# EdoardoBotta/RQ-VAE-Recommender

Measured on AMD Instinct MI355X. Metric: item-embeddings quantized/sec (RQ-VAE fwd+bwd), higher is better.
Workload: dtype f32 (MLP GEMMs f16x2-emulated)

## Files before the change

rq-vae-recommender_amd/csrc/gemm_split.hip:

```cpp
#include "rqhip_common.h"

namespace rqhip {

typedef float gs_f32x16 __attribute__((ext_vector_type(16)));
typedef float gs_f32x4 __attribute__((ext_vector_type(4)));
typedef float gs_f32x2 __attribute__((ext_vector_type(2)));
typedef __bf16 gs_bf16x8 __attribute__((ext_vector_type(8)));
typedef __bf16 gs_bf16x2 __attribute__((ext_vector_type(2)));
typedef _Float16 gs_f16x8 __attribute__((ext_vector_type(8)));
typedef _Float16 gs_f16x2 __attribute__((ext_vector_type(2)));
typedef unsigned gs_u32x2 __attribute__((ext_vector_type(2)));
typedef unsigned gs_u32x4 __attribute__((ext_vector_type(4)));
typedef int gs_i32x4 __attribute__((ext_vector_type(4)));

constexpr int kGsUB = 2;
constexpr int kGsK = 16;
constexpr int kGsColmaxLds = 1024;
constexpr int kGsTailWords = kWeightImageTailWords;

__device__ __forceinline__ void gs_split2(float a, float b, unsigned &h, unsigned &m, unsigned &l) {
    const gs_bf16x2 hh = __builtin_convertvector(gs_f32x2{a, b}, gs_bf16x2);
    h = __builtin_bit_cast(unsigned, hh);
    const float ra = a - __builtin_bit_cast(float, h << 16), rb = b - __builtin_bit_cast(float, h & 0xffff0000u);
    const gs_bf16x2 mm = __builtin_convertvector(gs_f32x2{ra, rb}, gs_bf16x2);
    m = __builtin_bit_cast(unsigned, mm);
    const float sa = ra - __builtin_bit_cast(float, m << 16), sb = rb - __builtin_bit_cast(float, m & 0xffff0000u);
    const gs_bf16x2 ll = __builtin_convertvector(gs_f32x2{sa, sb}, gs_bf16x2);
    l = __builtin_bit_cast(unsigned, ll);
}
__device__ __forceinline__ void gs_split2_f16(float a, float b, unsigned &h, unsigned &m) {
    const gs_f16x2 hh = __builtin_convertvector(gs_f32x2{a, b}, gs_f16x2);
    h = __builtin_bit_cast(unsigned, hh);
    const gs_f32x2 hf = __builtin_convertvector(hh, gs_f32x2);
    const gs_f16x2 mm = __builtin_convertvector(gs_f32x2{a - hf.x, b - hf.y}, gs_f16x2);
    m = __builtin_bit_cast(unsigned, mm);
}
constexpr int kGsF16Top = 14;
__device__ __forceinline__ int gs_exp_of_bits(unsigned b) {
    b &= 0x7fffffffu;
    const int e = (int)(b >> 23);
    return (b == 0u || e == 255) ? 0 : (e == 0 ? -126 : e - 127) - kGsF16Top;
}
__device__ __forceinline__ unsigned gs_abs_bits(float v) { return __builtin_bit_cast(unsigned, v) & 0x7fffffffu; }
__device__ __forceinline__ unsigned gs_umax(unsigned a, unsigned b) { return a > b ? a : b; }
__device__ __forceinline__ unsigned gs_half_wave_umax(unsigned v) {
    v = gs_umax(v, (unsigned)__builtin_amdgcn_update_dpp(0, (int)v, 0x111, 0xf, 0xf, true));
    v = gs_umax(v, (unsigned)__builtin_amdgcn_update_dpp(0, (int)v, 0x112, 0xf, 0xf, true));
    v = gs_umax(v, (unsigned)__builtin_amdgcn_update_dpp(0, (int)v, 0x114, 0xf, 0xf, true));
    v = gs_umax(v, (unsigned)__builtin_amdgcn_update_dpp(0, (int)v, 0x118, 0xf, 0xf, true));
    v = gs_umax(v, (unsigned)__builtin_amdgcn_update_dpp(0, (int)v, 0x142, 0xa, 0xf, true));
    return v;
}

constexpr int kImgCols = 4;
constexpr int kImgMaxJobs = 16;
struct ImageJob {
    const float *src;
    unsigned *image;
    int Nc, R, transpose, np;
    int block0;
};
struct ImageJobs {
    ImageJob j[kImgMaxJobs];
    int n;
};

__global__ __launch_bounds__(256) void weight_images_kernel(const ImageJobs jobs) {
    int ji = 0;
#pragma unroll 1
    for (int i = 1; i < jobs.n; ++i)
        if ((int)blockIdx.x >= jobs.j[i].block0) ji = i;
    const ImageJob job = jobs.j[ji];
    const int blk = (int)blockIdx.x - job.block0;
    const int Nc = job.Nc, R = job.R, np = job.np, n0 = blk * kImgCols;
    unsigned *tail = job.image + (size_t)(R / kGsK) * 2 * np * Nc * 4;
    if (blk == 0 && threadIdx.x < kGsTailWords) tail[threadIdx.x] = 0u;
    __shared__ unsigned s_max[kImgCols];
    if (threadIdx.x < kImgCols) s_max[threadIdx.x] = 0u;
    __syncthreads();
    const int pairs = R / 2, total = kImgCols * pairs;
    auto locate = [&](int idx, int &nl, int &rp) {
        if (job.transpose) { nl = idx % kImgCols; rp = idx / kImgCols; }
        else { rp = idx % pairs; nl = idx / pairs; }
    };
    auto fetch = [&](int nl, int rp, float &a, float &b) {
        const int n = n0 + nl, r = 2 * rp;
        a = job.transpose ? job.src[(size_t)r * Nc + n] : job.src[(size_t)n * R + r];
        b = job.transpose ? job.src[(size_t)(r + 1) * Nc + n] : job.src[(size_t)n * R + r + 1];
    };
    if (np == 2) {
        if (job.transpose) {
            __shared__ unsigned s_part[256];
            const int nl = threadIdx.x % kImgCols;
            unsigned m = 0u;
            for (int r = threadIdx.x / kImgCols; r < R; r += 256 / kImgCols) m = gs_umax(m, gs_abs_bits(job.src[(size_t)r * Nc + n0 + nl]));
            s_part[threadIdx.x] = m;
            __syncthreads();
            if (threadIdx.x < kImgCols) {
                for (int i = threadIdx.x + kImgCols; i < 256; i += kImgCols) m = gs_umax(m, s_part[i]);
                s_max[threadIdx.x] = m;
            }
        } else {
            const int lane = threadIdx.x & 63, nl = threadIdx.x >> 6;
            unsigned m = 0u;
            for (int rp = lane; rp < pairs; rp += 64) {
                const gs_f32x2 v = *reinterpret_cast<const gs_f32x2 *>(job.src + (size_t)(n0 + nl) * R + 2 * rp);
                m = gs_umax(m, gs_umax(gs_abs_bits(v.x), gs_abs_bits(v.y)));
            }
#pragma unroll
            for (int o = 32; o > 0; o >>= 1) m = gs_umax(m, (unsigned)__shfl_xor((int)m, o, 64));
            if (lane == 0) s_max[nl] = m;
        }
        __syncthreads();
        if (threadIdx.x < kImgCols) reinterpret_cast<int *>(tail + kGsTailWords)[n0 + threadIdx.x] = gs_exp_of_bits(s_max[threadIdx.x]);
    }
    for (int idx = threadIdx.x; idx < total; idx += 256) {
        int nl, rp;
        float a, b;
        locate(idx, nl, rp);
        fetch(nl, rp, a, b);
        const int n = n0 + nl, r = 2 * rp;
        unsigned h, m, l = 0u;
        if (np == 2) {
            const int e = gs_exp_of_bits(s_max[nl]);
            gs_split2_f16(ldexpf(a, -e), ldexpf(b, -e), h, m);
        } else {
            gs_split2(a, b, h, m, l);
        }
        const int s = r >> 4, half = (r >> 3) & 1, j2 = (r & 7) >> 1;
        const size_t base = ((size_t)(s * np) * 2 + half) * Nc + n;
        job.image[(base + 0 * 2 * (size_t)Nc) * 4 + j2] = h;
        job.image[(base + 1 * 2 * (size_t)Nc) * 4 + j2] = m;
        if (np == 3) job.image[(base + 2 * 2 * (size_t)Nc) * 4 + j2] = l;
    }
}

__global__ __launch_bounds__(256) void maxima_kernel(const float *__restrict__ A, const float *__restrict__ Y, float *__restrict__ out,
                                                     long long M, int R, unsigned *__restrict__ row_max, unsigned *__restrict__ col_max) {
    extern __shared__ unsigned mx_smem[];
    const int lane = threadIdx.x & 63, wave = threadIdx.x >> 6;
    if (col_max) {
        for (int c = threadIdx.x; c < R; c += 256) mx_smem[c] = 0u;
        __syncthreads();
    }
    constexpr int kQ = 4;
    for (int c0 = 0; c0 < R; c0 += 256 * kQ) {
    const int R4 = (R - c0 < 256 * kQ ? R - c0 : 256 * kQ) / 4;
    unsigned cm[kQ][4];
#pragma unroll
    for (int q = 0; q < kQ; ++q)
#pragma unroll
        for (int j = 0; j < 4; ++j) cm[q][j] = 0u;
    for (long long row = (long long)blockIdx.x * 4 + wave; row < M; row += (long long)gridDim.x * 4) {
        const gs_f32x4 *src = reinterpret_cast<const gs_f32x4 *>(A + (size_t)row * R + c0);
        const gs_f32x4 *ys = Y ? reinterpret_cast<const gs_f32x4 *>(Y + (size_t)row * R + c0) : nullptr;
        gs_f32x4 *dst = out ? reinterpret_cast<gs_f32x4 *>(out + (size_t)row * R + c0) : nullptr;
        unsigned rm = 0u;
#pragma unroll
        for (int q = 0; q < kQ; ++q) {
            const int i = lane + 64 * q;
            if (i >= R4) break;
            gs_f32x4 v = src[i];
            if (ys) {
                const gs_f32x4 y4 = ys[i];
                v.x = y4.x <= 0.0f ? 0.0f : v.x; v.y = y4.y <= 0.0f ? 0.0f : v.y;
                v.z = y4.z <= 0.0f ? 0.0f : v.z; v.w = y4.w <= 0.0f ? 0.0f : v.w;
                if (dst) dst[i] = v;
            }
#pragma unroll
            for (int j = 0; j < 4; ++j) {
                const unsigned b = gs_abs_bits(v[j]);
                rm = gs_umax(rm, b);
                cm[q][j] = gs_umax(cm[q][j], b);
            }
        }
        if (row_max) {
#pragma unroll
            for (int o = 32; o > 0; o >>= 1) rm = gs_umax(rm, (unsigned)__shfl_xor((int)rm, o, 64));
            if (lane == 0) row_max[row] = c0 == 0 ? rm : gs_umax(rm, row_max[row]);
        }
    }
    if (col_max) {
#pragma unroll
        for (int q = 0; q < kQ; ++q) {
            const int i = lane + 64 * q;
            if (i >= R4) break;
#pragma unroll
            for (int j = 0; j < 4; ++j) atomicMax(&mx_smem[c0 + 4 * i + j], cm[q][j]);
        }
    }
    }
    if (col_max) {
        __syncthreads();
        for (int c = threadIdx.x; c < R; c += 256)
            if (mx_smem[c]) atomicMax(col_max + c, mx_smem[c]);
    }
}

struct GemmSplitParams {
    const float *A;
    const unsigned *planes;
    float *C;
    long long M;
    int R, Nc;
    int n_col_tiles;
    unsigned n_big, n_tiles;
    int rt_big;
    unsigned *counter;
    int n_queues;
    int rt_fastest;
    int static_tiles;
    const float *X;
    float *rowsum;
    float row_scale;
    const unsigned *a_max;
    int a_parts;
    const int *b_exp;
    unsigned *c_rowmax, *c_colmax;
};

#ifndef GS_PROBE
#define GS_PROBE 0
#endif
#ifndef GS_PROLOGUE_ORDER
#define GS_PROLOGUE_ORDER 1
#endif
#ifndef GS_FAST_EPILOGUE
#define GS_FAST_EPILOGUE 1
#endif
#ifndef GS_REGION_PAD
#define GS_REGION_PAD 32
#endif

__device__ __forceinline__ unsigned gs_row16_umax(unsigned v) {
    v = gs_umax(v, (unsigned)__builtin_amdgcn_update_dpp(0, (int)v, 0x111, 0xf, 0xf, true));
    v = gs_umax(v, (unsigned)__builtin_amdgcn_update_dpp(0, (int)v, 0x112, 0xf, 0xf, true));
    v = gs_umax(v, (unsigned)__builtin_amdgcn_update_dpp(0, (int)v, 0x114, 0xf, 0xf, true));
    v = gs_umax(v, (unsigned)__builtin_amdgcn_update_dpp(0, (int)v, 0x118, 0xf, 0xf, true));
    return v;
}
__device__ __forceinline__ float gs_row16_sum(float v) {
    v = v + __builtin_bit_cast(float, __builtin_amdgcn_update_dpp(0, __builtin_bit_cast(int, v), 0x111, 0xf, 0xf, true));
    v = v + __builtin_bit_cast(float, __builtin_amdgcn_update_dpp(0, __builtin_bit_cast(int, v), 0x112, 0xf, 0xf, true));
    v = v + __builtin_bit_cast(float, __builtin_amdgcn_update_dpp(0, __builtin_bit_cast(int, v), 0x114, 0xf, 0xf, true));
    v = v + __builtin_bit_cast(float, __builtin_amdgcn_update_dpp(0, __builtin_bit_cast(int, v), 0x118, 0xf, 0xf, true));
    return v;
}

constexpr int kGsTS = 68;
__host__ __device__ constexpr size_t gs_epilogue_lds(int waves, int rows, int wn) { return (size_t)waves * 32 * kGsTS * 4 + (size_t)2 * wn * rows * 4; }

template <int EPI, int TA, int COLS, int NP, int WAVES>
__device__ __forceinline__ void gs_epilogue(const GemmSplitParams &p, gs_f32x16 (&acc)[TA][kGsUB], unsigned *sbuf, const int *s_aexp,
                                            unsigned *s_colmax, long long m0, int n0) {
    constexpr int kGsThreads = 64 * WAVES;
    constexpr int UB = kGsUB, WN = COLS / (32 * UB), WM = WAVES / WN, ROWS = WM * 32 * TA;
    static_assert(UB == 2, "a wave's tile is 64 columns wide");
    int tid = threadIdx.x;
    asm volatile("" : "+v"(tid));
    const int lane = tid & 63, wave = tid >> 6;
    const int il = lane & 31, h = lane >> 5;
    const int wm = wave / WN, wn = wave % WN;
    const int cl = lane & 15, rl = lane >> 4;
    float *tb = reinterpret_cast<float *>(sbuf) + (size_t)wave * 32 * kGsTS;
    float *red = reinterpret_cast<float *>(sbuf) + (size_t)WAVES * 32 * kGsTS;
    unsigned *mred = reinterpret_cast<unsigned *>(red) + WN * ROWS;
    const bool want_rowmax = p.c_rowmax != nullptr, want_colmax = p.c_colmax != nullptr;
    const int colw = n0 + 64 * wn + 4 * cl;
    gs_i32x4 ec = {0, 0, 0, 0};
    if (NP == 2) ec = *reinterpret_cast<const gs_i32x4 *>(p.b_exp + colw);
    unsigned cmx[4] = {0u, 0u, 0u, 0u};
#if GS_FAST_EPILOGUE
    if (NP == 2 && want_rowmax && want_colmax && m0 + ROWS <= p.M) {
        const size_t row0 = (size_t)(m0 + 32 * TA * wm + rl);
        float *cbase = p.C + row0 * p.Nc + colw;
        const float *xbase = EPI >= 2 ? p.X + row0 * p.Nc + colw : nullptr;
        unsigned *pad = reinterpret_cast<unsigned *>(tb) + il * kGsTS + 64 + h;
        gs_f32x4 xn[8];
        if (EPI >= 2) {
#pragma unroll
            for (int k = 0; k < 8; ++k) xn[k] = *reinterpret_cast<const gs_f32x4 *>(xbase + (size_t)(4 * k) * p.Nc);
        }
#pragma unroll
        for (int t = 0; t < TA; ++t) {
#pragma unroll
            for (int u = 0; u < UB; ++u)
#pragma unroll
                for (int g = 0; g < 4; ++g)
                    *reinterpret_cast<gs_f32x4 *>(tb + il * kGsTS + 32 * u + 8 * g + 4 * h) =
                        gs_f32x4{acc[t][u][4 * g], acc[t][u][4 * g + 1], acc[t][u][4 * g + 2], acc[t][u][4 * g + 3]};
            __builtin_amdgcn_fence(__ATOMIC_RELEASE, "wavefront");
            __builtin_amdgcn_wave_barrier();
            gs_f32x4 v8[8], x8[8];
            int er8[8];
#pragma unroll
            for (int k = 0; k < 8; ++k) {
                v8[k] = *reinterpret_cast<const gs_f32x4 *>(tb + (4 * k + rl) * kGsTS + 4 * cl);
                er8[k] = s_aexp[32 * TA * wm + 32 * t + 4 * k + rl];
            }
            if (EPI >= 2) {
#pragma unroll
                for (int k = 0; k < 8; ++k) x8[k] = xn[k];
                if (t + 1 < TA) {
#pragma unroll
                    for (int k = 0; k < 8; ++k) xn[k] = *reinterpret_cast<const gs_f32x4 *>(xbase + (size_t)(32 * (t + 1) + 4 * k) * p.Nc);
                }
            }
#pragma unroll
            for (int k = 0; k < 8; ++k) {
                const int rloc = 32 * TA * wm + 32 * t + 4 * k + rl;
                gs_f32x4 v = v8[k];
#pragma unroll
                for (int j = 0; j < 4; ++j) v[j] = ldexpf(v[j], er8[k] + ec[j]);
                const gs_f32x4 x4 = EPI >= 2 ? x8[k] : gs_f32x4{0.f, 0.f, 0.f, 0.f};
                if (EPI == 1) {
                    v.x = v.x < 0.0f ? 0.0f : v.x; v.y = v.y < 0.0f ? 0.0f : v.y;
                    v.z = v.z < 0.0f ? 0.0f : v.z; v.w = v.w < 0.0f ? 0.0f : v.w;
                }
                float sq = 0.0f;
                if (EPI == 2) {
#pragma unroll
                    for (int j = 0; j < 4; ++j) {
                        const float d = v[j] - x4[j];
                        sq = sq + d * d;
                        v[j] = (2.0f * d) * p.row_scale;
                    }
                }
                if (EPI == 3) {
                    v.x = x4.x <= 0.0f ? 0.0f : v.x; v.y = x4.y <= 0.0f ? 0.0f : v.y;
                    v.z = x4.z <= 0.0f ? 0.0f : v.z; v.w = x4.w <= 0.0f ? 0.0f : v.w;
                }
                unsigned rmx = 0u;
#pragma unroll
                for (int j = 0; j < 4; ++j) {
                    const unsigned bb = gs_abs_bits(v[j]);
                    rmx = gs_umax(rmx, bb);
                    cmx[j] = gs_umax(cmx[j], bb);
                }
                *reinterpret_cast<gs_f32x4 *>(cbase + (size_t)(32 * t + 4 * k) * p.Nc) = v;
                if (EPI == 2) {
                    const float s16 = gs_row16_sum(sq);
                    float *dst = cl == 15 ? red + wn * ROWS + rloc : reinterpret_cast<float *>(pad);
                    *dst = s16;
                }
                const unsigned m16 = gs_row16_umax(rmx);
                unsigned *dstm = cl == 15 ? mred + wn * ROWS + rloc : pad;
                *dstm = m16;
            }
            __builtin_amdgcn_fence(__ATOMIC_RELEASE, "wavefront");
            __builtin_amdgcn_wave_barrier();
        }
    } else
#endif
    {
    constexpr int kAux = 4, NQ = 8 * TA;
    gs_f32x4 xa[kAux];
    auto aux_of = [&](int q) {
        long long r = m0 + 32 * TA * wm + 4 * q + rl;
        r = r < p.M ? r : p.M - 1;
        return *reinterpret_cast<const gs_f32x4 *>(p.X + (size_t)r * p.Nc + colw);
    };
    if (EPI >= 2) {
#pragma unroll
        for (int q = 0; q < kAux; ++q) xa[q] = aux_of(q);
    }
#pragma unroll
    for (int t = 0; t < TA; ++t) {
#pragma unroll
        for (int u = 0; u < UB; ++u)
#pragma unroll
            for (int g = 0; g < 4; ++g)
                *reinterpret_cast<gs_f32x4 *>(tb + il * kGsTS + 32 * u + 8 * g + 4 * h) =
                    gs_f32x4{acc[t][u][4 * g], acc[t][u][4 * g + 1], acc[t][u][4 * g + 2], acc[t][u][4 * g + 3]};
        __builtin_amdgcn_fence(__ATOMIC_RELEASE, "wavefront");
        __builtin_amdgcn_wave_barrier();
#pragma unroll
        for (int k = 0; k < 8; ++k) {
            const int q = 8 * t + k;
            const int rloc = 32 * TA * wm + 32 * t + 4 * k + rl;
            const long long grow = m0 + rloc;
            gs_f32x4 v = *reinterpret_cast<const gs_f32x4 *>(tb + (4 * k + rl) * kGsTS + 4 * cl);
            if (NP == 2) {
                const int er = s_aexp[rloc];
#pragma unroll
                for (int j = 0; j < 4; ++j) v[j] = ldexpf(v[j], er + ec[j]);
            }
            gs_f32x4 x4 = {0.f, 0.f, 0.f, 0.f};
            if (EPI >= 2) {
                x4 = xa[q % kAux];
                if (q + kAux < NQ) xa[q % kAux] = aux_of(q + kAux);
            }
            if (EPI == 1) {
                v.x = v.x < 0.0f ? 0.0f : v.x; v.y = v.y < 0.0f ? 0.0f : v.y;
                v.z = v.z < 0.0f ? 0.0f : v.z; v.w = v.w < 0.0f ? 0.0f : v.w;
            }
            float sq = 0.0f;
            if (EPI == 2) {
#pragma unroll
                for (int j = 0; j < 4; ++j) {
                    const float d = v[j] - x4[j];
                    sq = sq + d * d;
                    v[j] = (2.0f * d) * p.row_scale;
                }
            }
            if (EPI == 3) {
                v.x = x4.x <= 0.0f ? 0.0f : v.x; v.y = x4.y <= 0.0f ? 0.0f : v.y;
                v.z = x4.z <= 0.0f ? 0.0f : v.z; v.w = x4.w <= 0.0f ? 0.0f : v.w;
            }
            unsigned rmx = 0u;
            if (grow < p.M) {
                if (want_rowmax | want_colmax) {
#pragma unroll
                    for (int j = 0; j < 4; ++j) {
                        const unsigned bb = gs_abs_bits(v[j]);
                        rmx = gs_umax(rmx, bb);
                        cmx[j] = gs_umax(cmx[j], bb);
                    }
                }
                *reinterpret_cast<gs_f32x4 *>(p.C + (size_t)grow * p.Nc + colw) = v;
            }
            if (EPI == 2) {
                const float s16 = gs_row16_sum(sq);
                if (cl == 15) red[wn * ROWS + rloc] = s16;
            }
            if (want_rowmax) {
                const unsigned m16 = gs_row16_umax(rmx);
                if (cl == 15) mred[wn * ROWS + rloc] = m16;
            }
        }
        __builtin_amdgcn_fence(__ATOMIC_RELEASE, "wavefront");
        __builtin_amdgcn_wave_barrier();
    }
    }
    if (want_colmax) {
#pragma unroll
        for (int j = 0; j < 4; ++j) {
            unsigned m = gs_umax(cmx[j], (unsigned)__shfl_xor((int)cmx[j], 16, 64));
            m = gs_umax(m, (unsigned)__shfl_xor((int)m, 32, 64));
            if (rl == 0 && m != 0u) {
                if (p.Nc <= kGsColmaxLds) atomicMax(&s_colmax[colw + j], m);
                else atomicMax(p.c_colmax + colw + j, m);
            }
        }
    }
    if (want_rowmax || EPI == 2) {
        __syncthreads();
        if (want_rowmax) {
            unsigned *dst = p.c_rowmax + (size_t)(n0 / (COLS > 256 ? 256 : COLS)) * p.M;
            for (int r = tid; r < ROWS; r += kGsThreads) {
                if (m0 + r >= p.M) continue;
                unsigned mx = mred[r];
#pragma unroll
                for (int w = 1; w < WN; ++w) mx = gs_umax(mx, mred[w * ROWS + r]);
                dst[m0 + r] = mx;
                if (COLS > 256) dst[p.M + m0 + r] = mx;
            }
        }
        if (EPI == 2) {
            for (int r = tid; r < ROWS; r += kGsThreads) {
                if (m0 + r >= p.M) continue;
                float sum = red[r];
#pragma unroll
                for (int w = 1; w < WN; ++w) sum = sum + red[w * ROWS + r];
                p.rowsum[(size_t)(n0 / COLS) * p.M + m0 + r] = sum;
            }
        }
    }
}

template <int EPI, int TA, int COLS, int NP, int WAVES>
__device__ __forceinline__ void gs_tile(const GemmSplitParams &p, unsigned *sbuf, int *s_aexp, unsigned *s_colmax, long long m0, int n0) {
    constexpr int kGsWaves = WAVES, kGsThreads = 64 * WAVES;
    constexpr int UB = kGsUB, WN = COLS / (32 * UB), WM = kGsWaves / WN;
    constexpr int ROWS = WM * 32 * TA, AQ = (ROWS * 4 + kGsThreads - 1) / kGsThreads;
    constexpr int PA = NP * 2 * ROWS * 4, PB = NP * 2 * COLS * 4;
    constexpr int BQ = (2 * NP * COLS + kGsThreads - 1) / kGsThreads;
    const int tid = threadIdx.x, lane = tid & 63, wave = tid >> 6;
    const int il = lane & 31, h = lane >> 5;
    const int wm = wave / WN, wn = wave % WN;
    const int n_stage = p.R / kGsK;
    constexpr int APASS = kGsThreads / 4;
    const int arow = tid >> 2, akq = tid & 3;
    constexpr bool kAllLive = (ROWS * 4) % kGsThreads == 0;
    bool a_live[AQ];
    const float *asrc[AQ];
    int a_e[AQ];
#pragma unroll
    for (int q = 0; q < AQ; ++q) {
        a_live[q] = kAllLive || arow + APASS * q < ROWS;
        long long arow_g = m0 + arow + APASS * q;
        arow_g = arow_g < p.M ? arow_g : p.M - 1;
        asrc[q] = p.A + (size_t)arow_g * p.R + 4 * akq;
        a_e[q] = 0;
        if (NP == 2) {
            unsigned mx = 0u;
            const unsigned *am = p.a_max + arow_g;
            for (int part = 0; part < p.a_parts; part += 4) {
                unsigned v[4];
#pragma unroll
                for (int j = 0; j < 4; ++j) v[j] = am[(size_t)(part + j < p.a_parts ? part + j : part) * p.M];
                mx = gs_umax(gs_umax(mx, gs_umax(v[0], v[1])), gs_umax(v[2], v[3]));
            }
            a_e[q] = gs_exp_of_bits(mx);
            if (a_live[q] && akq == 0) s_aexp[arow + APASS * q] = a_e[q];
        }
    }

    gs_f32x16 acc[TA][UB];
#pragma unroll
    for (int t = 0; t < TA; ++t)
#pragma unroll
        for (int u = 0; u < UB; ++u)
#pragma unroll
            for (int r = 0; r < 16; ++r) acc[t][u][r] = 0.0f;

    gs_f32x4 ra0[AQ], ra1[AQ];
    gs_u32x4 rb[BQ];
    auto fetchA = [&](int stage, gs_f32x4 *dst) {
        stage = stage < n_stage ? stage : n_stage - 1;
#pragma unroll
        for (int q = 0; q < AQ; ++q) dst[q] = *reinterpret_cast<const gs_f32x4 *>(asrc[q] + stage * kGsK);
    };
    auto fetchB = [&](int stage) {
        stage = stage < n_stage ? stage : n_stage - 1;
        const gs_u32x4 *img = reinterpret_cast<const gs_u32x4 *>(p.planes) + (size_t)stage * 2 * NP * p.Nc + n0;
#pragma unroll
        for (int q = 0; q < BQ; ++q) {
            const int e = tid + kGsThreads * q;
            if ((2 * NP * COLS) % kGsThreads != 0 && e >= 2 * NP * COLS) continue;
            rb[q] = img[(size_t)(e / COLS) * p.Nc + (e % COLS)];
        }
    };
    auto stash = [&](int buf, const gs_f32x4 *ra) {
        unsigned *dA = sbuf + buf * (PA + PB), *dB = dA + PA;
#pragma unroll
        for (int q = 0; q < AQ; ++q) {
            if (!kAllLive && !a_live[q]) continue;
            unsigned h01, m01, l01 = 0u, h23, m23, l23 = 0u;
            if (NP == 2) {
                gs_split2_f16(ldexpf(ra[q].x, -a_e[q]), ldexpf(ra[q].y, -a_e[q]), h01, m01);
                gs_split2_f16(ldexpf(ra[q].z, -a_e[q]), ldexpf(ra[q].w, -a_e[q]), h23, m23);
            } else {
                gs_split2(ra[q].x, ra[q].y, h01, m01, l01);
                gs_split2(ra[q].z, ra[q].w, h23, m23, l23);
            }
            unsigned *d = dA + (((akq >> 1) * ROWS) + arow + APASS * q) * 4 + 2 * (akq & 1);
            *reinterpret_cast<gs_u32x2 *>(d + 0 * 2 * ROWS * 4) = gs_u32x2{h01, h23};
            *reinterpret_cast<gs_u32x2 *>(d + 1 * 2 * ROWS * 4) = gs_u32x2{m01, m23};
            if (NP == 3) *reinterpret_cast<gs_u32x2 *>(d + 2 * 2 * ROWS * 4) = gs_u32x2{l01, l23};
        }
#pragma unroll
        for (int q = 0; q < BQ; ++q) {
            const int e = tid + kGsThreads * q;
            if ((2 * NP * COLS) % kGsThreads != 0 && e >= 2 * NP * COLS) continue;
            *reinterpret_cast<gs_u32x4 *>(dB + (size_t)e * 4) = rb[q];
        }
    };
    auto multiply = [&](int buf) {
        const gs_bf16x8 *aA = reinterpret_cast<const gs_bf16x8 *>(sbuf + buf * (PA + PB));
        const gs_bf16x8 *bB = reinterpret_cast<const gs_bf16x8 *>(sbuf + buf * (PA + PB) + PA);
        if constexpr (NP == 2) {
            gs_f16x8 fb[UB][2];
#pragma unroll
            for (int u = 0; u < UB; ++u)
#pragma unroll
                for (int pc = 0; pc < 2; ++pc)
                    fb[u][pc] = __builtin_bit_cast(gs_f16x8, bB[(pc * 2 + h) * COLS + wn * 32 * UB + 32 * u + il]);
#pragma unroll
            for (int t = 0; t < TA; ++t) {
                gs_f16x8 fa[2];
#pragma unroll
                for (int pc = 0; pc < 2; ++pc)
                    fa[pc] = __builtin_bit_cast(gs_f16x8, aA[(pc * 2 + h) * ROWS + wm * 32 * TA + 32 * t + il]);
#pragma unroll
                for (int u = 0; u < UB; ++u) {
                    gs_f32x16 c16 = acc[t][u];
                    c16 = __builtin_amdgcn_mfma_f32_32x32x16_f16(fb[u][0], fa[1], c16, 0, 0, 0);
                    c16 = __builtin_amdgcn_mfma_f32_32x32x16_f16(fb[u][1], fa[0], c16, 0, 0, 0);
                    c16 = __builtin_amdgcn_mfma_f32_32x32x16_f16(fb[u][0], fa[0], c16, 0, 0, 0);
                    acc[t][u] = c16;
                }
            }
        } else {
#pragma unroll
            for (int u = 0; u < UB; ++u) {
                gs_bf16x8 b[3];
#pragma unroll
                for (int pc = 0; pc < 3; ++pc) b[pc] = bB[(pc * 2 + h) * COLS + wn * 32 * UB + 32 * u + il];
#pragma unroll
                for (int t = 0; t < TA; ++t) {
                    gs_bf16x8 a[3];
#pragma unroll
                    for (int pc = 0; pc < 3; ++pc) a[pc] = aA[(pc * 2 + h) * ROWS + wm * 32 * TA + 32 * t + il];
                    gs_f32x16 c16 = acc[t][u];
                    c16 = __builtin_amdgcn_mfma_f32_32x32x16_bf16(b[1], a[1], c16, 0, 0, 0);
                    c16 = __builtin_amdgcn_mfma_f32_32x32x16_bf16(b[0], a[2], c16, 0, 0, 0);
                    c16 = __builtin_amdgcn_mfma_f32_32x32x16_bf16(b[2], a[0], c16, 0, 0, 0);
                    c16 = __builtin_amdgcn_mfma_f32_32x32x16_bf16(b[0], a[1], c16, 0, 0, 0);
                    c16 = __builtin_amdgcn_mfma_f32_32x32x16_bf16(b[1], a[0], c16, 0, 0, 0);
                    c16 = __builtin_amdgcn_mfma_f32_32x32x16_bf16(b[0], a[0], c16, 0, 0, 0);
                    acc[t][u] = c16;
                }
            }
        }
    };

#if GS_PROLOGUE_ORDER
    gs_f32x4 rp[AQ];
    fetchA(0, rp);
    fetchB(0);
    __builtin_amdgcn_sched_barrier(0);
    fetchA(1, ra1);
    __builtin_amdgcn_sched_barrier(0);
    stash(0, rp);
    __builtin_amdgcn_sched_barrier(0);
    fetchB(1);
    __builtin_amdgcn_sched_barrier(0);
    fetchA(2, ra0);
    __builtin_amdgcn_sched_barrier(0);
    __syncthreads();
#else
    fetchA(0, ra0);
    fetchB(0);
    fetchA(1, ra1);
    stash(0, ra0);
    fetchB(1);
    fetchA(2, ra0);
    __syncthreads();
#endif
    const int n_pair = n_stage & ~1;
    for (int c = 0; c < n_pair; c += 2) {
        stash(1, ra1);
        fetchB(c + 2);
        fetchA(c + 3, ra1);
        multiply(0);
        __syncthreads();
        stash(0, ra0);
        fetchB(c + 3);
        fetchA(c + 4, ra0);
        multiply(1);
        __syncthreads();
    }
    if (n_stage & 1) {
        multiply(0);
        __syncthreads();
    }

    gs_epilogue<EPI, TA, COLS, NP, WAVES>(p, acc, sbuf, s_aexp, s_colmax, m0, n0);
}

template <int EPI, int TA, int COLS = 256>
__device__ __forceinline__ void gs_tile2(const GemmSplitParams &p, unsigned *sbuf, int *s_aexp, unsigned *s_colmax, long long m0, int n0) {
    constexpr int WAVES = COLS / 64, UB = kGsUB, kThreads = 64 * WAVES;
    constexpr int ROWS = 32 * TA;
    constexpr int AQ = (ROWS * 4 + kThreads - 1) / kThreads;
    constexpr bool kAllLive = (ROWS * 4) % kThreads == 0;
    constexpr int kRegion = ROWS * 4 + GS_REGION_PAD;
    constexpr int PA = 4 * kRegion;
    const int tid = threadIdx.x, lane = tid & 63, wn = tid >> 6;
    const int il = lane & 31, h = lane >> 5;
    const int n_stage = p.R / kGsK;
    constexpr int APASS = kThreads / 4;
    const int arow = tid >> 2, akq = tid & 3;
    const float *asrc[AQ];
    int a_e[AQ];
    bool a_live[AQ];
#pragma unroll
    for (int q = 0; q < AQ; ++q) {
        a_live[q] = kAllLive || arow + APASS * q < ROWS;
        long long arow_g = m0 + arow + APASS * q;
        arow_g = arow_g < p.M ? arow_g : p.M - 1;
        asrc[q] = p.A + (size_t)arow_g * p.R + 4 * akq;
        unsigned mx = 0u;
        const unsigned *am = p.a_max + arow_g;
        for (int part = 0; part < p.a_parts; part += 4) {
            unsigned v[4];
#pragma unroll
            for (int j = 0; j < 4; ++j) v[j] = am[(size_t)(part + j < p.a_parts ? part + j : part) * p.M];
            mx = gs_umax(gs_umax(mx, gs_umax(v[0], v[1])), gs_umax(v[2], v[3]));
        }
        a_e[q] = gs_exp_of_bits(mx);
        if (a_live[q] && akq == 0) s_aexp[arow + APASS * q] = a_e[q];
    }

    gs_f32x16 acc[TA][UB];
#pragma unroll
    for (int t = 0; t < TA; ++t)
#pragma unroll
        for (int u = 0; u < UB; ++u)
#pragma unroll
            for (int r = 0; r < 16; ++r) acc[t][u][r] = 0.0f;

    const gs_u32x4 *bsrc = reinterpret_cast<const gs_u32x4 *>(p.planes) + (size_t)h * p.Nc + n0 + 64 * wn + il;
    const size_t b_stage = (size_t)4 * p.Nc, b_piece = (size_t)2 * p.Nc;
    gs_f32x4 ra0[AQ], ra1[AQ];
    gs_u32x4 fb0[UB][2], fb1[UB][2];
    auto fetchA = [&](int stage, gs_f32x4 *dst) {
        stage = stage < n_stage ? stage : n_stage - 1;
#pragma unroll
        for (int q = 0; q < AQ; ++q) {
            if (GS_PROBE & 4) dst[q] = gs_f32x4{1.f + stage, 2.f, 3.f, 4.f};
            else if (GS_PROBE & 64) {
                size_t o = (size_t)m0 * p.R + (size_t)stage * ROWS * kGsK + (size_t)(tid + kThreads * q) * 4;
                if (o + 4 > (size_t)p.M * p.R) o = 0;
                dst[q] = *reinterpret_cast<const gs_f32x4 *>(p.A + o);
            }
            else dst[q] = *reinterpret_cast<const gs_f32x4 *>(asrc[q] + stage * kGsK);
        }
    };
    auto fetchB = [&](int stage, gs_u32x4 (*dst)[2]) {
        stage = stage < n_stage ? stage : n_stage - 1;
        const gs_u32x4 *img = bsrc + (size_t)stage * b_stage;
#pragma unroll
        for (int u = 0; u < UB; ++u)
#pragma unroll
            for (int pc = 0; pc < 2; ++pc) {
                if (GS_PROBE & 8) dst[u][pc] = gs_u32x4{(unsigned)stage, 1u, 2u, 3u};
                else dst[u][pc] = img[(size_t)pc * b_piece + 32 * u];
            }
    };
    auto stash = [&](int buf, const gs_f32x4 *ra) {
        unsigned *dA = sbuf + buf * PA;
        if (GS_PROBE & 2) return;
#pragma unroll
        for (int q = 0; q < AQ; ++q) {
            if (!kAllLive && !a_live[q]) continue;
            unsigned h01, m01, h23, m23;
            gs_split2_f16(ldexpf(ra[q].x, -a_e[q]), ldexpf(ra[q].y, -a_e[q]), h01, m01);
            gs_split2_f16(ldexpf(ra[q].z, -a_e[q]), ldexpf(ra[q].w, -a_e[q]), h23, m23);
            unsigned *d = dA + (akq >> 1) * kRegion + (arow + APASS * q) * 4 + 2 * (akq & 1);
            *reinterpret_cast<gs_u32x2 *>(d) = gs_u32x2{h01, h23};
            *reinterpret_cast<gs_u32x2 *>(d + 2 * kRegion) = gs_u32x2{m01, m23};
        }
    };
    auto loadA = [&](int buf, int t, gs_f16x8 *fa) {
        const gs_u32x4 *aA = reinterpret_cast<const gs_u32x4 *>(sbuf + buf * PA);
#pragma unroll
        for (int pc = 0; pc < 2; ++pc) {
            if (GS_PROBE & 32) fa[pc] = gs_f16x8{(_Float16)(float)(t + buf), 1, 2, 3, 4, 5, 6, 7};
            else fa[pc] = __builtin_bit_cast(gs_f16x8, aA[(pc * 2 + h) * (kRegion / 4) + 32 * t + il]);
        }
    };
    auto multiply = [&](int buf, const gs_u32x4 (*fbr)[2]) {
        gs_f16x8 fa[2][2];
        loadA(buf, 0, fa[0]);
#pragma unroll
        for (int t = 0; t < TA; ++t) {
            if (t + 1 < TA) loadA(buf, t + 1, fa[(t + 1) & 1]);
#pragma unroll
            for (int u = 0; u < UB; ++u) {
                const gs_f16x8 bh = __builtin_bit_cast(gs_f16x8, fbr[u][0]), bm = __builtin_bit_cast(gs_f16x8, fbr[u][1]);
                gs_f32x16 c16 = acc[t][u];
                if (GS_PROBE & 16) {
                    c16[0] += (float)bh[0] + (float)bm[1] + (float)fa[t & 1][0][2] + (float)fa[t & 1][1][3];
                } else {
                    c16 = __builtin_amdgcn_mfma_f32_32x32x16_f16(bh, fa[t & 1][1], c16, 0, 0, 0);
                    c16 = __builtin_amdgcn_mfma_f32_32x32x16_f16(bm, fa[t & 1][0], c16, 0, 0, 0);
                    c16 = __builtin_amdgcn_mfma_f32_32x32x16_f16(bh, fa[t & 1][0], c16, 0, 0, 0);
                }
                acc[t][u] = c16;
            }
        }
    };

#if GS_PROLOGUE_ORDER
    gs_f32x4 rp[AQ];
    fetchA(0, rp);
    __builtin_amdgcn_sched_barrier(0);
    fetchA(1, ra1);
    __builtin_amdgcn_sched_barrier(0);
    fetchB(0, fb0);
    __builtin_amdgcn_sched_barrier(0);
    fetchA(2, ra0);
    __builtin_amdgcn_sched_barrier(0);
    fetchB(1, fb1);
    __builtin_amdgcn_sched_barrier(0);
    stash(0, rp);
    __syncthreads();
#else
    fetchA(0, ra0);
    fetchB(0, fb0);
    fetchA(1, ra1);
    stash(0, ra0);
    fetchB(1, fb1);
    fetchA(2, ra0);
    __syncthreads();
#endif
    const int n_pair = n_stage & ~1;
    for (int c = 0; c < n_pair; c += 2) {
        stash(1, ra1);
        fetchA(c + 3, ra1);
        multiply(0, fb0);
        fetchB(c + 2, fb0);
        if (!(GS_PROBE & 1)) __syncthreads();
        stash(0, ra0);
        fetchA(c + 4, ra0);
        multiply(1, fb1);
        fetchB(c + 3, fb1);
        if (!(GS_PROBE & 1)) __syncthreads();
    }
    if (n_stage & 1) {
        multiply(0, fb0);
        __syncthreads();
    }
    gs_epilogue<EPI, TA, COLS, 2, WAVES>(p, acc, sbuf, s_aexp, s_colmax, m0, n0);
}

template <int EPI, int COLS, int NP, int WAVES, int BIGROWS = 0>
__global__ __launch_bounds__(64 * WAVES, BIGROWS ? 4 : 2) void gemm_split_kernel(const GemmSplitParams p) {
    constexpr int kGsThreads = 64 * WAVES;
    constexpr int kSmallRows = (WAVES / (COLS / 64)) * 32;
    constexpr int kBigRows = BIGROWS ? BIGROWS : 32 * WAVES;
    extern __shared__ __attribute__((aligned(16))) char gs_smem[];
    unsigned *sbuf = reinterpret_cast<unsigned *>(gs_smem);
    __shared__ unsigned s_tile;
    __shared__ int s_aexp[kBigRows];
    __shared__ unsigned s_colmax[kGsColmaxLds];
    const int tid = threadIdx.x;
    const bool lds_colmax = p.c_colmax != nullptr && p.Nc <= kGsColmaxLds;
    if (lds_colmax)
        for (int c = tid; c < p.Nc; c += kGsThreads) s_colmax[c] = 0u;
    unsigned static_next = blockIdx.x;
    for (;;) {
        __syncthreads();
        unsigned tile;
        if (p.static_tiles) {
            tile = static_next;
            static_next += gridDim.x;
            if (tile >= p.n_tiles) break;
        } else {
            if (tid == 0) s_tile = atomicAdd(p.counter, 1u);
            __syncthreads();
            tile = s_tile;
            if (tile >= p.n_tiles) {
                if (tid == 0 && atomicAdd(p.counter + 1, 1u) == gridDim.x - 1) {
                    p.counter[0] = 0u;
                    p.counter[1] = 0u;
                }
                break;
            }
        }
        if (tile < p.n_big) {
            const int ct = (int)(tile % (unsigned)p.n_col_tiles), rt = (int)(tile / (unsigned)p.n_col_tiles);
            gs_tile<EPI, kBigRows / kSmallRows, COLS, NP, WAVES>(p, sbuf, s_aexp, s_colmax, (long long)rt * kBigRows, ct * COLS);
        } else {
            const unsigned st = tile - p.n_big;
            const int ct = (int)(st % (unsigned)p.n_col_tiles), rt = (int)(st / (unsigned)p.n_col_tiles);
            gs_tile<EPI, 1, COLS, NP, WAVES>(p, sbuf, s_aexp, s_colmax, (long long)p.rt_big * kBigRows + (long long)rt * kSmallRows, ct * COLS);
        }
    }
    if (lds_colmax) {
        __syncthreads();
        for (int c = tid; c < p.Nc; c += kGsThreads)
            if (s_colmax[c]) atomicMax(p.c_colmax + c, s_colmax[c]);
    }
}

constexpr int kGsQueues = 8;
template <int EPI, int COLS = 256, int SMALL_TA = 2>
__global__ __launch_bounds__(COLS, COLS == 256 ? 2 : 1) void gemm_f16_kernel(const GemmSplitParams p) {
    constexpr int kThreads = COLS, kBigRows = 128, kSmallRows = 32 * SMALL_TA;
    constexpr unsigned kSmallBit = 0x80000000u, kNone = 0xffffffffu;
    extern __shared__ __attribute__((aligned(16))) char gs_smem[];
    unsigned *sbuf = reinterpret_cast<unsigned *>(gs_smem);
    __shared__ unsigned s_tile;
    __shared__ int s_aexp[kBigRows];
    __shared__ unsigned s_colmax[kGsColmaxLds];
    const int tid = threadIdx.x;
    const bool lds_colmax = p.c_colmax != nullptr && p.Nc <= kGsColmaxLds;
    if (lds_colmax)
        for (int c = tid; c < p.Nc; c += kThreads) s_colmax[c] = 0u;
    const unsigned nct = (unsigned)p.n_col_tiles;
    const unsigned rt_big = p.n_big / nct, rt_small = (p.n_tiles - p.n_big) / nct;
    const int nq = p.n_queues;
    const int xcd = (int)(blockIdx.x % (unsigned)nq);
    if (p.static_tiles) {
        for (unsigned tile = blockIdx.x; tile < p.n_tiles; tile += gridDim.x) {
            __syncthreads();
            if (tile < p.n_big) {
                const int ct = (int)(tile % nct), rt = (int)(tile / nct);
                gs_tile2<EPI, kBigRows / 32, COLS>(p, sbuf, s_aexp, s_colmax, (long long)rt * kBigRows, ct * COLS);
            } else {
                const unsigned st = tile - p.n_big;
                const int ct = (int)(st % nct), rt = (int)(st / nct);
                gs_tile2<EPI, kSmallRows / 32, COLS>(p, sbuf, s_aexp, s_colmax, (long long)p.rt_big * kBigRows + (long long)rt * kSmallRows, ct * COLS);
            }
        }
        if (lds_colmax) {
            __syncthreads();
            for (int c = tid; c < p.Nc; c += kThreads)
                if (s_colmax[c]) atomicMax(p.c_colmax + c, s_colmax[c]);
        }
        return;
    }
    int big_skip = 0, small_skip = 0;
    for (;;) {
        __syncthreads();
        if (tid == 0) {
            unsigned t = kNone;
            for (; big_skip < nq; ++big_skip) {
                const unsigned q = (unsigned)((xcd + big_skip) % nq);
                const unsigned j = atomicAdd(p.counter + q, 1u);
                const unsigned rt = (j / nct) * (unsigned)nq + q;
                if (rt < rt_big) { t = rt * nct + j % nct; break; }
            }
            if (t == kNone) {
                for (; small_skip < nq; ++small_skip) {
                    const unsigned q = (unsigned)((xcd + small_skip) % nq);
                    const unsigned j = atomicAdd(p.counter + kGsQueues + q, 1u);
                    const unsigned rt = (j / nct) * (unsigned)nq + q;
                    if (rt < rt_small) { t = (rt * nct + j % nct) | kSmallBit; break; }
                }
            }
            s_tile = t;
        }
        __syncthreads();
        const unsigned tile = s_tile;
        if (tile == kNone) {
            if (tid == 0 && atomicAdd(p.counter + 2 * kGsQueues, 1u) == gridDim.x - 1) {
                for (int i = 0; i <= 2 * kGsQueues; ++i) p.counter[i] = 0u;
            }
            break;
        }
        if (!(tile & kSmallBit)) {
            const int ct = p.rt_fastest ? (int)(tile / rt_big) : (int)(tile % nct), rt = p.rt_fastest ? (int)(tile % rt_big) : (int)(tile / nct);
            gs_tile2<EPI, kBigRows / 32, COLS>(p, sbuf, s_aexp, s_colmax, (long long)rt * kBigRows, ct * COLS);
        } else {
            const unsigned st = tile & ~kSmallBit;
            const int ct = p.rt_fastest ? (int)(st / rt_small) : (int)(st % nct), rt = p.rt_fastest ? (int)(st % rt_small) : (int)(st / nct);
            gs_tile2<EPI, kSmallRows / 32, COLS>(p, sbuf, s_aexp, s_colmax, (long long)p.rt_big * kBigRows + (long long)rt * kSmallRows, ct * COLS);
        }
    }
    if (lds_colmax) {
        for (int c = tid; c < p.Nc; c += kThreads)
            if (s_colmax[c]) atomicMax(p.c_colmax + c, s_colmax[c]);
    }
}

__global__ __launch_bounds__(256) void recon_rows_finish_kernel(const float *__restrict__ rowsum, int nct, long long M,
                                                                float *__restrict__ out) {
    const long long m = (long long)blockIdx.x * 256 + threadIdx.x;
    if (m >= M) return;
    float s = rowsum[m];
    for (int c = 1; c < nct; ++c) s = s + rowsum[(size_t)c * M + m];
    out[m] = s;
}

}

using namespace rqhip;

static int gs_cols(int Nc) { return Nc % 256 == 0 ? 256 : 128; }
static int gs_np(int arith) { return arith == RQHIP_SPLIT_F16X2 ? 2 : arith == RQHIP_SPLIT_BF16X3 ? 3 : 0; }
extern "C" int rqhip_gemm_split_supported(int Nc, int R) { return (Nc > 0 && R > 0 && Nc % 128 == 0 && R % kGsK == 0) ? 1 : 0; }

extern "C" size_t rqhip_weight_image_bytes(int Nc, int R, int arith) {
    const int np = gs_np(arith);
    if (!np || !rqhip_gemm_split_supported(Nc, R)) return 0;
    return (size_t)(R / kGsK) * 2 * np * Nc * 16 + kGsTailWords * 4 + (np == 2 ? (size_t)Nc * sizeof(int) : 0);
}
extern "C" size_t rqhip_weight_planes_bytes(int Nc, int R) { return rqhip_weight_image_bytes(Nc, R, RQHIP_SPLIT_BF16X3); }

extern "C" int rqhip_weight_images(const rqhip_image_job *jobs, int n_jobs, rqhip_stream_t stream) {
    if (n_jobs < 0 || (n_jobs > 0 && !jobs)) {
        set_error("weight_images: bad job list");
        return RQHIP_EARG;
    }
    hipStream_t s = reinterpret_cast<hipStream_t>(stream);
    for (int first = 0; first < n_jobs; first += kImgMaxJobs) {
        ImageJobs batch;
        batch.n = n_jobs - first < kImgMaxJobs ? n_jobs - first : kImgMaxJobs;
        int blocks = 0;
        for (int i = 0; i < batch.n; ++i) {
            const rqhip_image_job &j = jobs[first + i];
            const int Nc = j.transpose ? j.cols : j.rows, R = j.transpose ? j.rows : j.cols;
            const size_t need = rqhip_weight_image_bytes(Nc, R, j.arith);
            if (!j.w || !j.image || need == 0 || j.image_bytes < need || (reinterpret_cast<uintptr_t>(j.image) & 15u) != 0) {
                set_error("weight_images: job %d: bad arguments or unsupported shape (Nc = %d must be a multiple of 128, R = %d of 16, "
                          "image of rqhip_weight_image_bytes, 16-byte aligned)", first + i, Nc, R);
                return RQHIP_EARG;
            }
            ImageJob &d = batch.j[i];
            d.src = j.w; d.image = reinterpret_cast<unsigned *>(j.image); d.Nc = Nc; d.R = R; d.transpose = j.transpose ? 1 : 0;
            d.np = gs_np(j.arith); d.block0 = blocks;
            blocks += Nc / kImgCols;
        }
        hipLaunchKernelGGL(weight_images_kernel, dim3((unsigned)blocks), dim3(256), 0, s, batch);
        RQ_CHECK_LAUNCH("weight_images_kernel");
    }
    return RQHIP_OK;
}

extern "C" int rqhip_weight_planes(const float *w, int rows, int cols, int transpose, void *planes, size_t planes_bytes,
                                   rqhip_stream_t stream) {
    rqhip_image_job j;
    j.w = w; j.rows = rows; j.cols = cols; j.transpose = transpose; j.arith = RQHIP_SPLIT_BF16X3; j.image = planes; j.image_bytes = planes_bytes;
    return rqhip_weight_images(&j, 1, stream);
}

extern "C" int rqhip_maxima(const float *A, const float *Y, float *masked_out, int64_t M, int R, unsigned *row_max, unsigned *col_max,
                            rqhip_stream_t stream) {
    auto al16 = [](const void *q) { return (reinterpret_cast<uintptr_t>(q) & 15u) == 0; };
    if (M < 0 || R <= 0 || (R % 4) != 0 || R > 16384 || (M > 0 && !A) || (masked_out && !Y) || !al16(A) || !al16(Y) || !al16(masked_out)) {
        set_error("maxima: bad arguments (R = %d must be a multiple of 4, at most 16384; 16-byte aligned rows; masked_out needs Y)", R);
        return RQHIP_EARG;
    }
    if (M == 0 || (!row_max && !col_max && !masked_out)) return RQHIP_OK;
    long long blocks = (M + 3) / 4;
    const long long cap = (long long)cu_count() * 8;
    if (blocks > cap) blocks = cap;
    hipStream_t s = reinterpret_cast<hipStream_t>(stream);
    profile_begin(s, RQHIP_PROF_MAXIMA, 0.0, (double)M * R * 4 * ((Y ? 2 : 1) + (masked_out ? 1 : 0)));
    hipLaunchKernelGGL(maxima_kernel, dim3((unsigned)blocks), dim3(256), col_max ? (size_t)R * 4 : 0, s, A, Y, masked_out, (long long)M, R,
                       row_max, col_max);
    profile_end(s);
    RQ_CHECK_LAUNCH("maxima_kernel");
    return RQHIP_OK;
}

extern "C" size_t rqhip_gemm_split_recon_workspace_bytes(int64_t M, int Nc) {
    return (M > 0 && Nc > 0 && Nc % 256 == 0) ? (size_t)(Nc / 256) * (size_t)M * sizeof(float) : 0;
}

extern "C" int rqhip_gemm_split_ex(const rqhip_gemm_args *a, rqhip_stream_t stream) {
    if (!a) {
        set_error("gemm_split: null argument block");
        return RQHIP_EARG;
    }
    const int np = gs_np(a->arith), epi = a->epilogue;
    const int64_t M = a->M;
    const int R = a->R, Nc = a->Nc;
    if (!np || M < 0 || !a->image || (M > 0 && (!a->A || !a->C)) || !rqhip_gemm_split_supported(Nc, R) || epi < 0 || epi > 3) {
        set_error("gemm_split: bad arguments or unsupported shape (Nc = %d, R = %d, arithmetic %d, epilogue %d)", Nc, R, a->arith, epi);
        return RQHIP_EARG;
    }
    auto al16 = [](const void *q) { return (reinterpret_cast<uintptr_t>(q) & 15u) == 0; };
    if (!al16(a->A) || !al16(a->C) || !al16(a->image) || !al16(a->aux) || (R % 4) != 0) {
        set_error("gemm_split: pointers must be 16-byte aligned");
        return RQHIP_EARG;
    }
    if (M > 0 && np == 2 && (!a->a_row_max || a->a_row_parts < 1)) {
        set_error("gemm_split: RQHIP_SPLIT_F16X2 needs the row maxima of A (a_row_max from rqhip_maxima or from the epilogue that wrote A)");
        return RQHIP_EARG;
    }
    if (M > 0 && epi >= RQHIP_EPI_RECON && !a->aux) {
        set_error("gemm_split: epilogue %d needs aux (X / Y, [M, Nc])", epi);
        return RQHIP_EARG;
    }
    const int cols = gs_cols(Nc);
    if (epi == RQHIP_EPI_RECON && M > 0 && (cols != 256 || !a->loss_rows || !a->workspace ||
                                           a->workspace_bytes < rqhip_gemm_split_recon_workspace_bytes(M, Nc))) {
        set_error("gemm_split: the reconstruction-loss epilogue needs Nc %% 256 == 0 (Nc = %d), loss_rows and a workspace of "
                  "rqhip_gemm_split_recon_workspace_bytes", Nc);
        return RQHIP_EARG;
    }
    if (M == 0) return RQHIP_OK;
    hipStream_t s = reinterpret_cast<hipStream_t>(stream);
    GemmSplitParams p;
    p.A = a->A; p.planes = reinterpret_cast<const unsigned *>(a->image); p.C = a->C; p.M = M; p.R = R; p.Nc = Nc;
    p.X = a->aux; p.rowsum = reinterpret_cast<float *>(a->workspace); p.row_scale = a->row_scale;
    p.a_max = a->a_row_max; p.a_parts = a->a_row_parts;
    p.c_rowmax = a->c_row_max; p.c_colmax = a->c_col_max;
    p.n_queues = a->tile_rows == -8 ? kGsQueues : 1;
    p.rt_fastest = a->tile_rows == -2 ? 1 : 0;
    p.static_tiles = (a->tile_rows == -12 || a->tile_rows == -8 || a->tile_rows == -2) ? 0 : 1;
    p.counter = const_cast<unsigned *>(p.planes) + (size_t)(R / kGsK) * 2 * np * Nc * 4;
    p.b_exp = reinterpret_cast<const int *>(p.counter + kGsTailWords);
    const int cus = cu_count();
    const bool tile2 = np == 2 && cols == 256;
    const bool wide = tile2 && a->tile_rows == -5 && Nc % 512 == 0 && epi != RQHIP_EPI_RECON;
    const bool occ4 = tile2 && a->tile_rows == -6 && epi != RQHIP_EPI_RECON;
    const int waves = (np == 3 || wide || occ4) ? 8 : 4;
    const int big_rows = (wide || occ4) ? 128 : 32 * waves;
    int small_rows = tile2 ? 64 : (waves / (cols / 64)) * 32;
    p.n_col_tiles = Nc / (wide ? 512 : cols);
    const long long slots = (long long)cus * ((waves == 4 || occ4) ? 2 : 1);
    const long long rt_all = (M + big_rows - 1) / big_rows;
    long long rt_big = ((rt_all * p.n_col_tiles) / slots) * slots / p.n_col_tiles;
    if (rt_big * big_rows > M) rt_big = M / big_rows;
    bool all_big = (rt_all * p.n_col_tiles) % slots > (3 * slots) / 10 && rt_all * p.n_col_tiles >= slots;
    bool tiny = false;
    if (tile2 && !wide && a->tile_rows == -9) {
        const long long left_rows = M - rt_big * big_rows;
        if (left_rows > 0) {
            auto rounds = [&](int h) { return ((left_rows + h - 1) / h * p.n_col_tiles + slots - 1) / slots; };
            const double c_big = (double)rounds(128) * 1.0, c_small = (double)rounds(64) * 0.72, c_tiny = (double)rounds(32) * 0.56;
            tiny = c_tiny < c_small && c_tiny < c_big;
            all_big = !tiny && c_big <= c_small && rt_all * p.n_col_tiles >= slots;
            if (tiny) small_rows = 32;
        }
    }
    if (all_big) rt_big = rt_all;
    if (tile2 && !wide && (a->tile_rows == -10 || a->tile_rows == -11)) {
        rt_big = 0;
        tiny = a->tile_rows == -11;
        small_rows = tiny ? 32 : 64;
    }
    if (!tile2 && (a->tile_rows == 256 || a->tile_rows == 128)) rt_big = rt_all;
    if (!tile2 && (a->tile_rows == 64 || a->tile_rows == 32)) rt_big = 0;
    const long long rem_rows = M - rt_big * big_rows > 0 ? M - rt_big * big_rows : 0;
    const long long rt_small = (rem_rows + small_rows - 1) / small_rows;
    p.rt_big = (int)rt_big;
    p.n_big = (unsigned)(rt_big * p.n_col_tiles);
    p.n_tiles = p.n_big + (unsigned)(rt_small * p.n_col_tiles);
    size_t lds = (tile2 && !occ4) ? (size_t)2 * 4 * (128 * 4 + 32) * 4 : (size_t)2 * (np * 2 * (big_rows + cols) * 16);
// ... 63 lines not shown
```

Baseline: 40.27 million.

## Overlap A-tile f16 splitting with MFMA and simplify epilogue addressing

Splits the stash step into a register-only hi/lo f16 split and a separate LDS store. The split of the next A stage now runs inside the multiply loop, between MFMA groups, and the first LDS fragment load is hoisted ahead of the store, with sched_barrier masks fencing the schedule. The goal is to hide the VALU split cost behind matrix work. The epilogue also switches to 32-bit byte-offset addressing for C/X quads and sends non-writer lanes' reduction values to a dedicated dump area instead of a pad in the tile buffer. This adds register pressure (two sets of split registers live at once) and a little more LDS.

```diff
diff --git a/rq-vae-recommender_amd/csrc/gemm_split.hip b/rq-vae-recommender_amd/csrc/gemm_split.hip
--- a/rq-vae-recommender_amd/csrc/gemm_split.hip
+++ b/rq-vae-recommender_amd/csrc/gemm_split.hip
@@ -248,7 +248,10 @@
 }
 
 constexpr int kGsTS = 68;
-__host__ __device__ constexpr size_t gs_epilogue_lds(int waves, int rows, int wn) { return (size_t)waves * 32 * kGsTS * 4 + (size_t)2 * wn * rows * 4; }
+constexpr int kGsDump = 128 + 4;
+__host__ __device__ constexpr size_t gs_epilogue_lds(int waves, int rows, int wn) {
+    return (size_t)waves * 32 * kGsTS * 4 + (size_t)2 * wn * rows * 4 + (size_t)kGsDump * 4;
+}
 
 template <int EPI, int TA, int COLS, int NP, int WAVES>
 __device__ __forceinline__ void gs_epilogue(const GemmSplitParams &p, gs_f32x16 (&acc)[TA][kGsUB], unsigned *sbuf, const int *s_aexp,
@@ -272,14 +275,19 @@
     unsigned cmx[4] = {0u, 0u, 0u, 0u};
 #if GS_FAST_EPILOGUE
     if (NP == 2 && want_rowmax && want_colmax && m0 + ROWS <= p.M) {
-        const size_t row0 = (size_t)(m0 + 32 * TA * wm + rl);
-        float *cbase = p.C + row0 * p.Nc + colw;
-        const float *xbase = EPI >= 2 ? p.X + row0 * p.Nc + colw : nullptr;
-        unsigned *pad = reinterpret_cast<unsigned *>(tb) + il * kGsTS + 64 + h;
+        static_assert(32 * TA + 4 <= kGsDump, "the dump words take a wave's row quads");
+        const unsigned lane_off = (unsigned)(((32 * TA * wm + rl) * p.Nc + 64 * wn + 4 * cl) * 4);
+        auto quad_at = [&](const float *base, int q4) {
+            const char *u = reinterpret_cast<const char *>(base + ((size_t)m0 + q4) * p.Nc + n0);
+            return reinterpret_cast<gs_f32x4 *>(const_cast<char *>(u) + lane_off);
+        };
+        unsigned *dump = mred + WN * ROWS;
+        unsigned *mrow = cl == 15 ? mred + wn * ROWS + 32 * TA * wm + rl : dump + rl;
+        float *rrow = cl == 15 ? red + wn * ROWS + 32 * TA * wm + rl : reinterpret_cast<float *>(dump) + rl;
         gs_f32x4 xn[8];
         if (EPI >= 2) {
 #pragma unroll
-            for (int k = 0; k < 8; ++k) xn[k] = *reinterpret_cast<const gs_f32x4 *>(xbase + (size_t)(4 * k) * p.Nc);
+            for (int k = 0; k < 8; ++k) xn[k] = *quad_at(p.X, 4 * k);
         }
 #pragma unroll
         for (int t = 0; t < TA; ++t) {
@@ -303,12 +311,11 @@
                 for (int k = 0; k < 8; ++k) x8[k] = xn[k];
                 if (t + 1 < TA) {
 #pragma unroll
-                    for (int k = 0; k < 8; ++k) xn[k] = *reinterpret_cast<const gs_f32x4 *>(xbase + (size_t)(32 * (t + 1) + 4 * k) * p.Nc);
+                    for (int k = 0; k < 8; ++k) xn[k] = *quad_at(p.X, 32 * (t + 1) + 4 * k);
                 }
             }
 #pragma unroll
             for (int k = 0; k < 8; ++k) {
-                const int rloc = 32 * TA * wm + 32 * t + 4 * k + rl;
                 gs_f32x4 v = v8[k];
 #pragma unroll
                 for (int j = 0; j < 4; ++j) v[j] = ldexpf(v[j], er8[k] + ec[j]);
@@ -337,15 +344,9 @@
                     rmx = gs_umax(rmx, bb);
                     cmx[j] = gs_umax(cmx[j], bb);
                 }
-                *reinterpret_cast<gs_f32x4 *>(cbase + (size_t)(32 * t + 4 * k) * p.Nc) = v;
-                if (EPI == 2) {
-                    const float s16 = gs_row16_sum(sq);
-                    float *dst = cl == 15 ? red + wn * ROWS + rloc : reinterpret_cast<float *>(pad);
-                    *dst = s16;
-                }
-                const unsigned m16 = gs_row16_umax(rmx);
-                unsigned *dstm = cl == 15 ? mred + wn * ROWS + rloc : pad;
-                *dstm = m16;
+                *quad_at(p.C, 32 * t + 4 * k) = v;
+                if (EPI == 2) rrow[32 * t + 4 * k] = gs_row16_sum(sq);
+                mrow[32 * t + 4 * k] = gs_row16_umax(rmx);
             }
             __builtin_amdgcn_fence(__ATOMIC_RELEASE, "wavefront");
             __builtin_amdgcn_wave_barrier();
@@ -719,8 +720,7 @@
                 else dst[u][pc] = img[(size_t)pc * b_piece + 32 * u];
             }
     };
-    auto stash = [&](int buf, const gs_f32x4 *ra) {
-        unsigned *dA = sbuf + buf * PA;
+    auto split_regs = [&](const gs_f32x4 *ra, gs_u32x4 *sp) {
         if (GS_PROBE & 2) return;
 #pragma unroll
         for (int q = 0; q < AQ; ++q) {
@@ -728,11 +728,21 @@
             unsigned h01, m01, h23, m23;
             gs_split2_f16(ldexpf(ra[q].x, -a_e[q]), ldexpf(ra[q].y, -a_e[q]), h01, m01);
             gs_split2_f16(ldexpf(ra[q].z, -a_e[q]), ldexpf(ra[q].w, -a_e[q]), h23, m23);
+            sp[q] = gs_u32x4{h01, h23, m01, m23};
+        }
+    };
+    auto store_lds = [&](int buf, const gs_u32x4 *sp) {
+        unsigned *dA = sbuf + buf * PA;
+        if (GS_PROBE & 2) return;
+#pragma unroll
+        for (int q = 0; q < AQ; ++q) {
+            if (!kAllLive && !a_live[q]) continue;
             unsigned *d = dA + (akq >> 1) * kRegion + (arow + APASS * q) * 4 + 2 * (akq & 1);
-            *reinterpret_cast<gs_u32x2 *>(d) = gs_u32x2{h01, h23};
-            *reinterpret_cast<gs_u32x2 *>(d + 2 * kRegion) = gs_u32x2{m01, m23};
-        }
-    };
+            *reinterpret_cast<gs_u32x2 *>(d) = gs_u32x2{sp[q].x, sp[q].y};
+            *reinterpret_cast<gs_u32x2 *>(d + 2 * kRegion) = gs_u32x2{sp[q].z, sp[q].w};
+        }
+    };
+    gs_u32x4 sp0[AQ], sp1[AQ];
     auto loadA = [&](int buf, int t, gs_f16x8 *fa) {
         const gs_u32x4 *aA = reinterpret_cast<const gs_u32x4 *>(sbuf + buf * PA);
 #pragma unroll
@@ -741,12 +751,14 @@
             else fa[pc] = __builtin_bit_cast(gs_f16x8, aA[(pc * 2 + h) * (kRegion / 4) + 32 * t + il]);
         }
     };
-    auto multiply = [&](int buf, const gs_u32x4 (*fbr)[2]) {
-        gs_f16x8 fa[2][2];
-        loadA(buf, 0, fa[0]);
+    constexpr int kGsBlockFence = 0x2 | 0x4 | 0x10 | 0x20 | 0x40 | 0x400;
+    gs_f16x8 fa[2][2];
+    auto multiply = [&](int buf, const gs_u32x4 (*fbr)[2], auto &&between) {
 #pragma unroll
         for (int t = 0; t < TA; ++t) {
+            if (t > 0) __builtin_amdgcn_sched_barrier(kGsBlockFence);
             if (t + 1 < TA) loadA(buf, t + 1, fa[(t + 1) & 1]);
+            if (t == (TA > 1 ? 1 : 0)) between();
 #pragma unroll
             for (int u = 0; u < UB; ++u) {
                 const gs_f16x8 bh = __builtin_bit_cast(gs_f16x8, fbr[u][0]), bm = __builtin_bit_cast(gs_f16x8, fbr[u][1]);
@@ -775,32 +787,43 @@
     __builtin_amdgcn_sched_barrier(0);
     fetchB(1, fb1);
     __builtin_amdgcn_sched_barrier(0);
-    stash(0, rp);
+    split_regs(rp, sp0);
+    store_lds(0, sp0);
+    split_regs(ra1, sp1);
     __syncthreads();
 #else
     fetchA(0, ra0);
     fetchB(0, fb0);
     fetchA(1, ra1);
-    stash(0, ra0);
+    split_regs(ra0, sp0);
+    store_lds(0, sp0);
     fetchB(1, fb1);
     fetchA(2, ra0);
+    split_regs(ra1, sp1);
     __syncthreads();
 #endif
     const int n_pair = n_stage & ~1;
     for (int c = 0; c < n_pair; c += 2) {
-        stash(1, ra1);
+        loadA(0, 0, fa[0]);
+        __builtin_amdgcn_sched_barrier(kGsBlockFence);
+        store_lds(1, sp1);
         fetchA(c + 3, ra1);
-        multiply(0, fb0);
+        multiply(0, fb0, [&] { split_regs(ra0, sp0); });
         fetchB(c + 2, fb0);
         if (!(GS_PROBE & 1)) __syncthreads();
-        stash(0, ra0);
+        __builtin_amdgcn_sched_barrier(0);
+        loadA(1, 0, fa[0]);
+        __builtin_amdgcn_sched_barrier(kGsBlockFence);
+        store_lds(0, sp0);
         fetchA(c + 4, ra0);
-        multiply(1, fb1);
+        multiply(1, fb1, [&] { split_regs(ra1, sp1); });
         fetchB(c + 3, fb1);
         if (!(GS_PROBE & 1)) __syncthreads();
+        __builtin_amdgcn_sched_barrier(0);
     }
     if (n_stage & 1) {
-        multiply(0, fb0);
+        loadA(0, 0, fa[0]);
+        multiply(0, fb0, [] {});
         __syncthreads();
     }
     gs_epilogue<EPI, TA, COLS, 2, WAVES>(p, acc, sbuf, s_aexp, s_colmax, m0, n0);
```

Result: no change. 40.48 million (median of 6 runs) (+0.5%).
